# Jamie725/Multimodal-Object-Detection-via-Probabilistic-Ensembling

Measured on AMD Instinct MI355X. Metric: RGB+T frame-pairs/sec (FLIR-aligned 640x512, two R101-FPN detectors + ProbEn), higher is better.
Workload: dtype f16; 1 GPU; configs[2]: FLIR RGB + thermal two-detector ProbEn (probEn/v-avg), batch 32 per GPU, R101-FPN x2, 640x512 -> 800x1000 (padded 800x1024), K=3, random-init weights; batch_per_gpu=32, input_residency=frames resident in HBM before the timed region (no H2D inside it), schedule=two detector streams, staggered by res3, batches back to back

## Files before the change

include/proben_hip.h:

```cpp
#ifndef PROBEN_HIP_H
#define PROBEN_HIP_H

#include <stddef.h>
#include <stdint.h>

#ifdef __cplusplus
extern "C" {
#endif

#define PE_OK 0
#define PE_ERR_INVALID_ARG (-1)
#define PE_ERR_UNSUPPORTED (-2)
#define PE_ERR_HIP (-3)

#define PE_SCORE_PROBEN 0
#define PE_SCORE_AVG 1
#define PE_SCORE_MAX 2
#define PE_SCORE_PROBEN_BINARY 3
#define PE_SCORE_PROBEN_LOGP 4
#define PE_BOX_VAVG 0
#define PE_BOX_SAVG 1
#define PE_BOX_AVG 2
#define PE_BOX_ARGMAX 3

// ... 87 lines not shown
#define PE_POOL_NLL_MAX_BLOCKS 1024
int pe_proben_fuse_batch_pooled(const double* boxes, const double* scores, const double* log_probs,
                                const double* variances, const int32_t* classes, const int32_t* row_source,
                                const int32_t* offsets, const int32_t* row_counts, const int32_t* passthrough, int32_t num_images,
                                int32_t num_classes, int32_t max_rows_per_image, int32_t box_mode, double iou_thresh, double frame_w,
                                double frame_h, const double* log_prior,
                                const double* pool_weights,
                                int32_t num_detectors, double* out_boxes, float* out_scores, float* out_classes, int32_t* out_keep,
                                int32_t* out_counts, int32_t* out_cluster , void* stream);
int pe_proben_pack_pooled(const float* const* det_boxes_host, const float* const* det_scores_host,
                          const int32_t* const* det_classes_host, const float* const* det_probs_host,
                          const float* const* det_logits_host, const float* const* det_vars_host,
                          const int32_t* const* det_counts_host, const double* temperatures_host,
                          const double* var_scales_host , int32_t num_detectors, int32_t num_images,
                          int32_t det_stride, int32_t num_classes, int32_t max_class, int32_t row_stride, double* out_boxes,
                          double* out_scores, double* out_probs, double* out_log_probs , double* out_vars,
                          int32_t* out_classes, int32_t* out_offsets, int32_t* out_counts, int32_t* out_single_source,
                          int32_t* out_source, void* stream);
int pe_pool_nll(const double* log_probs, const int32_t* row_source, int64_t num_rows, int32_t num_columns,
                const int32_t* member_rows, int64_t num_members, const int32_t* cluster_offsets, const int32_t* labels,
                int32_t num_clusters, const double* log_prior , const double* weights_host, int32_t num_candidates,
                int32_t num_detectors, double* workspace, double* out, int32_t* out_flags , void* stream);

int pe_proben_fuse_batch_posterior(const double* boxes, const double* scores, const double* log_probs,
                                   const double* variances, const int32_t* classes, const int32_t* row_source,
                                   const int32_t* offsets, const int32_t* row_counts, const int32_t* passthrough, int32_t num_images,
                                   int32_t num_classes, int32_t max_rows_per_image, int32_t box_mode, double iou_thresh, double frame_w,
                                   double frame_h, const double* log_prior,
                                   const double* pool_weights,
                                   int32_t num_detectors, double* out_boxes, float* out_scores, float* out_classes, int32_t* out_keep,
                                   int32_t* out_counts, int32_t* out_cluster ,
                                   double* out_log_posterior , double* out_vars ,
                                   int32_t* out_members , void* stream);

#define PE_PRESENCE_MAX_DETECTORS 4
#define PE_BIAS_NLL_MAX_COLUMNS 16
#define PE_BIAS_NLL_MAX_BLOCKS 1024
int pe_proben_fuse_batch_presence(const double* boxes, const double* scores, const double* log_probs,
                                  const double* variances, const int32_t* classes, const int32_t* row_source,
                                  const int32_t* offsets, const int32_t* row_counts, const int32_t* passthrough, int32_t num_images,
                                  int32_t num_classes, int32_t max_rows_per_image, int32_t box_mode, double iou_thresh, double frame_w,
                                  double frame_h, const double* log_prior,
                                  const double* pool_weights,
                                  const double* presence,
                                  int32_t num_detectors, double* out_boxes, float* out_scores, float* out_classes, int32_t* out_keep,
                                  int32_t* out_counts, int32_t* out_cluster ,
                                  double* out_log_posterior , double* out_vars ,
                                  int32_t* out_members ,
                                  int32_t* out_pattern , void* stream);
int pe_bias_nll(const double* base, const int32_t* labels, int32_t num_clusters, int32_t num_columns, const double* candidates_host,
                int32_t num_candidates, double* workspace, double* out, int32_t* out_flags , void* stream);

#define PE_BOX_CORR_MAX_DETECTORS PE_PRESENCE_MAX_DETECTORS
#define PE_BOX_PAIR_MAX_BLOCKS 1024
int pe_box_gls_batch(const double* boxes, const double* variances, const int32_t* row_source, const int32_t* cluster,
                     const int32_t* offsets, const int32_t* row_counts , const int32_t* counts, int32_t num_images,
                     int32_t max_rows_per_image, const double* correlation, int32_t num_detectors, double* out_boxes ,
                     double* out_vars , void* stream);
int pe_box_pair_stats(const double* boxes, const double* variances, const int32_t* row_source, int64_t num_rows,
                      const int32_t* member_rows, int64_t num_members, const int32_t* cluster_offsets, const int32_t* cluster_match,
                      int32_t num_clusters, const double* gt_boxes, int64_t num_gt, int32_t num_detectors,
                      const float* bbox_reg_weights_host , double* workspace, double* out ,
                      int32_t* out_flags , void* stream);

int pe_conv2d_nhwc_f16(const void* input, const void* weight, const float* bias, const void* residual,
                       void* output, int32_t N, int32_t H, int32_t W, int32_t Cin, int32_t Cout,
                       int32_t kernel, int32_t stride, int32_t relu, int32_t residual_mode,
                       int32_t res_h, int32_t res_w, int32_t out_f32, int32_t cout_store,
                       int32_t out_stride, void* stream);

int pe_conv_wd_supported(int32_t kernel, int32_t stride, int32_t H, int32_t W, int32_t Cin, int32_t Cout);
int pe_conv_wd_pack_weights(const void* weight, void* packed, int32_t Cout, int32_t Cin, int32_t kernel, void* stream);
int pe_conv3x3_wd_f16(const void* input, const void* packed_weight, const float* bias, void* output, int32_t N,
                      int32_t H, int32_t W, int32_t Cin, int32_t Cout, int32_t relu, int32_t out_stride, void* stream);
int pe_conv_wd_pack_tail(const void* weight, void* packed, int32_t tail_cout, int32_t C, void* stream);
int pe_bottleneck_tail_wd_f16(const void* input, const void* packed_weight3x3, const float* bias3x3, const void* packed_tail,
                              const float* tail_bias, const void* residual, void* output, int32_t N, int32_t H, int32_t W,
                              int32_t Cin, int32_t tail_cout, void* stream);
size_t pe_bneck64_packed_bytes(int32_t has_shortcut_conv, int32_t has_next);
int pe_bneck64_pack(const void* w2, const void* w3, const void* wsc, const void* w1n, void* packed, void* stream);
int pe_bneck64_f16(const void* t1, const void* shortcut_src, const void* packed, const float* bias2, const float* bias3,
                   const float* bias_sc, const float* bias1n, void* out, void* t1_next, int32_t N, int32_t H, int32_t W,
                   int32_t has_shortcut_conv, int32_t has_next, void* stream);
int pe_conv_wd_pack_head(const void* head_weight, void* packed, int32_t rows, int32_t C, void* stream);
int pe_conv3x3_wd_rpn_head_f16(const void* input, const void* packed_weight, const float* bias, const void* packed_head,
                               const float* head_bias16, float* head_out, int32_t N, int32_t H, int32_t W, int32_t Cin,
                               void* stream);

int pe_preprocess_pack(const void* src, int32_t src_kind, int32_t src_h, int32_t src_w, int32_t src_c,
                       int32_t ch0, int32_t nch, int32_t flip_rgb, int32_t dst_h, int32_t dst_w,
                       int32_t pad_h, int32_t pad_w, const float* mean_host, const float* std_host,
                       void* dst, void* stream);
int pe_preprocess_pack_batch(const void* src, int32_t num_images, int32_t src_kind, int32_t src_h, int32_t src_w,
                             int32_t src_c, int32_t ch0, int32_t nch, int32_t flip_rgb, int32_t dst_h, int32_t dst_w,
                             int32_t pad_h, int32_t pad_w, const float* mean_host, const float* std_host, void* dst,
                             void* stream);
int pe_preprocess_pack_pil_u8(const void* src, int32_t num_images, int32_t src_h, int32_t src_w, int32_t src_c,
                              int32_t ch0, int32_t nch, int32_t flip_rgb, int32_t dst_h, int32_t dst_w, int32_t pad_h,
                              int32_t pad_w, const float* mean_host, const float* std_host, const int32_t* xtab,
                              int32_t xk, const int32_t* ytab, int32_t yk, void* dst, void* stream);
int pe_fusion_input_pack(const void* thermal, const void* rgb, int32_t num_images, int32_t th_h, int32_t th_w, int32_t rgb_h,
                         int32_t rgb_w, int32_t ch0, int32_t nch, int32_t dst_h, int32_t dst_w, int32_t pad_h, int32_t pad_w,
                         int32_t pad_multiple, const float* mean_host, const float* std_host, void* dst, void* stream);
int pe_maxpool3x3s2_nhwc(const void* in, void* out, int32_t N, int32_t H, int32_t W, int32_t C, void* stream);
int pe_subsample2_nhwc(const void* in, void* out, int32_t N, int32_t H, int32_t W, int32_t C, void* stream);
int pe_stem_conv7x7_maxpool_f16(const void* x, const void* w_packed, const float* bias, void* out, int32_t N,
                                int32_t H, int32_t W, void* stream);

#define PE_NMS_TRICK 0
#define PE_NMS_CLASS 1
size_t pe_nms_scratch_bytes(int32_t B, int32_t n_max);
int pe_nms_batched(const float* boxes, const float* scores, const int32_t* idxs, const int32_t* counts,
                   const uint8_t* valid, int32_t B, int32_t n_max, float iou_thresh, int32_t mode,
                   int32_t max_out, int32_t* out_keep, int32_t* out_counts, void* scratch,
                   size_t scratch_bytes, void* stream);

int pe_rpn_select_topk(const float* const* level_heads_host, const int32_t* level_hw_host,
                       const int32_t* level_stride_host, const float* cell_anchors_host,
                       int32_t num_levels, int32_t N, int32_t head_stride, int32_t pre_nms_topk,
                       const int32_t* image_hw, float scale_clamp, float* cand_boxes, float* cand_scores,
                       int32_t* cand_level, uint8_t* cand_valid, int32_t cand_per_image, void* scratch,
                       size_t scratch_bytes, void* stream);
size_t pe_rpn_scratch_bytes(const int32_t* level_hw_host, int32_t num_levels, int32_t N);
int pe_gather_boxes(const float* boxes, const float* scores, const int32_t* keep, const int32_t* counts,
                    int32_t N, int32_t n_in, int32_t max_out, float* out_boxes, float* out_scores,
                    void* stream);

int pe_box2box_apply_deltas(const float* deltas, const float* boxes, int32_t N, int32_t k, const float* weights_host,
                            float scale_clamp, float* out, void* stream);
int pe_grid_anchors(const float* cell_anchors, int32_t num_cell_anchors, int32_t H, int32_t W, int32_t stride,
                    float offset, float* out, void* stream);

int pe_sgd_momentum_f32(float* params, const float* grads, float* momentum_buf, void* fp16_shadow, int64_t n, float lr,
                        float momentum, float weight_decay, float grad_scale, int32_t first_step, void* stream);

int pe_roi_align_nhwc(const void* const* feats_host, const int32_t* feat_hw_host, const float* scales_host,
                      int32_t num_levels, int32_t N, int32_t C, int32_t dtype, const float* rois,
                      int32_t rois_have_batch_index, int32_t num_rois, int32_t per_image,
                      const int32_t* counts, int32_t pooled_h, int32_t pooled_w, int32_t sampling_ratio,
                      int32_t aligned, void* output, int32_t* out_level, void* stream);

int pe_roi_align_nhwc_sorted(const void* const* feats_host, const int32_t* feat_hw_host, const float* scales_host,
                             int32_t num_levels, int32_t N, int32_t C, int32_t dtype, const float* boxes, int32_t per_image,
                             const int32_t* counts, int32_t pooled_h, int32_t pooled_w, int32_t sampling_ratio,
                             int32_t aligned, void* output, int32_t* out_level, int32_t* order_workspace, void* stream);

int pe_roi_align_backward_nhwc(const void* grad_output, int32_t dtype, const int32_t* feat_hw_host, const float* scales_host,
                               int32_t num_levels, int32_t N, int32_t C, const float* rois, int32_t rois_have_batch_index,
                               int32_t num_rois, int32_t per_image, const int32_t* counts, int32_t pooled_h,
                               int32_t pooled_w, int32_t sampling_ratio, int32_t aligned, float* const* grad_feats_host,
                               void* stream);

int pe_boxhead_candidates(const float* head, int32_t head_stride, int32_t N, int32_t per_image,
                          int32_t num_classes, const int32_t* prop_counts, const float* proposals,
                          const int32_t* image_hw, const float* reg_weights_host, float scale_clamp,
                          float score_thresh, int32_t cand_max, float* cand_boxes, float* cand_scores,
                          int32_t* cand_class, int32_t* cand_rows, int32_t* cand_counts, int32_t* cand_total,
                          float* probs, void* stream);
int pe_boxhead_finalize(const float* head, int32_t head_stride, int32_t N, int32_t per_image,
                        int32_t num_classes, int32_t cand_max, int32_t max_det, int32_t fix_vars,
                        const float* probs, const float* cand_boxes, const float* cand_scores,
                        const int32_t* cand_class, const int32_t* cand_rows, const int32_t* keep,
                        const int32_t* keep_counts, const int32_t* image_hw, const int32_t* out_hw,
                        float* det_boxes, float* det_scores, int32_t* det_classes, float* det_logits,
                        float* det_probs, float* det_vars, int32_t* det_rows, int32_t* det_counts,
                        void* stream);
// ... 12 lines not shown
```

multimodal-object-detection-via-probabilistic-ensembling_amd/_lib.py:

```python
import ctypes
import os

import torch

_PKG = os.path.dirname(os.path.abspath(__file__))
LIB_PATH = os.path.join(_PKG, "libproben_hip.so")
_lib = None

c_void_p, c_int, c_double, c_float = ctypes.c_void_p, ctypes.c_int32, ctypes.c_double, ctypes.c_float
c_size_t = ctypes.c_size_t

SIGNATURES = {
    "pe_version": [],
    "pe_proben_pack_detections": [c_void_p] * 6 + [c_int] * 6 + [c_void_p] * 9,
    "pe_proben_pack_logits": [c_void_p] * 6 + [c_int] * 6 + [c_void_p] * 9,
    "pe_proben_pack_log_posteriors": [c_void_p] * 6 + [c_int] * 6 + [c_void_p] * 10,
    "pe_log_softmax": [c_void_p, ctypes.c_int64, c_int, c_double, c_void_p, c_void_p],
    "pe_proben_fuse_batch_logp": [c_void_p] * 8 + [c_int] * 4 + [c_double] * 3 + [c_void_p] * 6 + [c_void_p],
    "pe_calibrated_softmax": [c_void_p, ctypes.c_int64, c_int, c_double, c_void_p, c_void_p],
    "pe_temperature_nll": [c_void_p, c_void_p, ctypes.c_int64, c_int, c_void_p, c_int, c_void_p, c_void_p, c_void_p, c_void_p],
    "pe_match_ground_truth": [c_void_p] * 6 + [c_int, c_double, c_int] + [c_void_p] * 4,
    "pe_variance_stats": [c_void_p] * 4 + [ctypes.c_int64, ctypes.c_int64, c_void_p, c_double] + [c_void_p] * 4,
    "pe_proben_pack_calibrated": [c_void_p] * 9 + [c_int] * 6 + [c_void_p] * 10,
    "pe_proben_fuse_batch_pooled": [c_void_p] * 9 + [c_int] * 4 + [c_double] * 3 + [c_void_p] * 2 + [c_int] + [c_void_p] * 6 + [c_void_p],
    "pe_proben_fuse_batch_posterior": [c_void_p] * 9 + [c_int] * 4 + [c_double] * 3 + [c_void_p] * 2 + [c_int] + [c_void_p] * 9 + [c_void_p],
    "pe_proben_fuse_batch_presence": [c_void_p] * 9 + [c_int] * 4 + [c_double] * 3 + [c_void_p] * 3 + [c_int] + [c_void_p] * 10 + [c_void_p],
    "pe_bias_nll": [c_void_p, c_void_p, c_int, c_int, c_void_p, c_int, c_void_p, c_void_p, c_void_p, c_void_p],
    "pe_box_gls_batch": [c_void_p] * 7 + [c_int, c_int, c_void_p, c_int] + [c_void_p] * 3,
    "pe_box_pair_stats": [c_void_p] * 3 + [ctypes.c_int64, c_void_p, ctypes.c_int64, c_void_p, c_void_p, c_int, c_void_p, ctypes.c_int64,
                          c_int] + [c_void_p] * 5,
    "pe_proben_pack_pooled": [c_void_p] * 9 + [c_int] * 6 + [c_void_p] * 11,
    "pe_pool_nll": [c_void_p, c_void_p, ctypes.c_int64, c_int, c_void_p, ctypes.c_int64, c_void_p, c_void_p, c_int, c_void_p, c_void_p,
                    c_int, c_int, c_void_p, c_void_p, c_void_p, c_void_p],
    "pe_reliability_logits": [c_void_p] * 3 + [ctypes.c_int64, c_int, c_double, c_int] + [c_void_p] * 5,
    "pe_reliability_scores": [c_void_p] * 2 + [ctypes.c_int64, c_int] + [c_void_p] * 5,
    "pe_proben_fuse_batch": [c_void_p] * 8 + [c_int] * 5 + [c_double] * 3 + [c_void_p] * 5 + [c_void_p],
    "pe_conv2d_nhwc_f16": [c_void_p] * 5 + [c_int] * 14 + [c_void_p],
    "pe_conv_wd_supported": [c_int] * 6,
    "pe_conv_wd_pack_weights": [c_void_p] * 2 + [c_int] * 3 + [c_void_p],
    "pe_conv3x3_wd_f16": [c_void_p] * 4 + [c_int] * 7 + [c_void_p],
    "pe_conv_wd_pack_tail": [c_void_p] * 2 + [c_int] * 2 + [c_void_p],
    "pe_bottleneck_tail_wd_f16": [c_void_p] * 7 + [c_int] * 5 + [c_void_p],
    "pe_bneck64_packed_bytes": [c_int] * 2,
    "pe_bneck64_pack": [c_void_p] * 6,
    "pe_bneck64_f16": [c_void_p] * 9 + [c_int] * 5 + [c_void_p],
    "pe_conv_wd_pack_head": [c_void_p] * 2 + [c_int] * 2 + [c_void_p],
    "pe_conv3x3_wd_rpn_head_f16": [c_void_p] * 6 + [c_int] * 4 + [c_void_p],
    "pe_preprocess_pack": [c_void_p] + [c_int] * 11 + [c_void_p] * 4,
    "pe_preprocess_pack_batch": [c_void_p] + [c_int] * 12 + [c_void_p] * 4,
    "pe_preprocess_pack_pil_u8": [c_void_p] + [c_int] * 11 + [c_void_p] * 2 + [c_void_p, c_int, c_void_p, c_int] + [c_void_p] * 2,
    "pe_fusion_input_pack": [c_void_p] * 2 + [c_int] * 12 + [c_void_p] * 4,
    "pe_maxpool3x3s2_nhwc": [c_void_p] * 2 + [c_int] * 4 + [c_void_p],
    "pe_subsample2_nhwc": [c_void_p] * 2 + [c_int] * 4 + [c_void_p],
    "pe_stem_conv7x7_maxpool_f16": [c_void_p] * 4 + [c_int] * 3 + [c_void_p],
    "pe_nms_scratch_bytes": [c_int, c_int],
    "pe_nms_batched": [c_void_p] * 5 + [c_int, c_int, c_float, c_int, c_int] + [c_void_p] * 3 + [c_size_t, c_void_p],
    "pe_rpn_select_topk": [c_void_p] * 4 + [c_int] * 4 + [c_void_p, c_float] + [c_void_p] * 4 + [c_int, c_void_p, c_size_t, c_void_p],
    "pe_rpn_scratch_bytes": [c_void_p, c_int, c_int],
    "pe_box2box_apply_deltas": [c_void_p] * 2 + [c_int] * 2 + [c_void_p, c_float, c_void_p, c_void_p],
    "pe_grid_anchors": [c_void_p, c_int, c_int, c_int, c_int, c_float, c_void_p, c_void_p],
    "pe_gather_boxes": [c_void_p] * 4 + [c_int] * 3 + [c_void_p] * 3,
    "pe_roi_align_nhwc": [c_void_p] * 3 + [c_int] * 4 + [c_void_p] + [c_int] * 3 + [c_void_p] + [c_int] * 4 + [c_void_p] * 3,
    "pe_roi_align_nhwc_sorted": [c_void_p] * 3 + [c_int] * 4 + [c_void_p] + [c_int] + [c_void_p] + [c_int] * 4 + [c_void_p] * 4,
    "pe_sgd_momentum_f32": [c_void_p] * 4 + [ctypes.c_int64] + [ctypes.c_float] * 4 + [c_int, c_void_p],
    "pe_roi_align_backward_nhwc": [c_void_p, c_int, c_void_p, c_void_p, c_int, c_int, c_int, c_void_p, c_int, c_int, c_int, c_void_p, c_int, c_int, c_int, c_int, c_void_p, c_void_p],
    "pe_boxhead_candidates": [c_void_p, c_int, c_int, c_int, c_int] + [c_void_p] * 4 + [c_float, c_float, c_int] + [c_void_p] * 8,
    "pe_cocoeval_bbox": [c_void_p] * 6 + [ctypes.c_int64] + [c_void_p] * 4 + [ctypes.c_int64, c_int, c_int, c_void_p, c_int,
                         c_void_p, c_int, c_void_p, c_int, c_void_p, c_int, c_int, c_void_p, c_void_p],
    "pe_boxhead_finalize": [c_void_p] + [c_int] * 7 + [c_void_p] * 18,
}
_RESTYPE = {"pe_last_error": ctypes.c_char_p, "pe_nms_scratch_bytes": ctypes.c_size_t, "pe_rpn_scratch_bytes": ctypes.c_size_t,
             "pe_bneck64_packed_bytes": ctypes.c_size_t}


TEST_HOOKS = {"pe_test_set_conv_policy": [c_int, c_int], "pe_test_set_wd9_mode": [c_int], "pe_test_wd9_takes": [c_int] * 5, "pe_test_wd9_head_takes": [c_int] * 3, "pe_test_set_wd9_wgs": [c_int, c_int], "pe_test_set_ring_wgs": [c_int], "pe_test_set_roi_fast": [c_int], "pe_test_set_nms_presorted": [c_int]}


class HipLibraryError(RuntimeError):
    pass


def lib():
    global _lib
    if _lib is None:
        if not os.path.exists(LIB_PATH):
            raise HipLibraryError(
                f"{LIB_PATH} is missing: run `python -c 'import __graft_entry__ as g; g.build()'` "
                "(hipcc --offload-arch=gfx950).  proben_amd has no CPU fallback.")
        L = ctypes.CDLL(LIB_PATH)
        L.pe_last_error.restype = ctypes.c_char_p
        L.pe_last_error.argtypes = []
        for name, args in SIGNATURES.items():
            fn = getattr(L, name)
            fn.argtypes = args
            fn.restype = _RESTYPE.get(name, ctypes.c_int)
        _lib = L
    return _lib


LAB_HOOKS = {"pe_test_set_ring_ablation": [c_int]}


def test_hooks():
    L = lib()
    for name, args in LAB_HOOKS.items():
        if hasattr(L, name):
            getattr(L, name).argtypes, getattr(L, name).restype = args, ctypes.c_int
    for name, args in TEST_HOOKS.items():
        fn = getattr(L, name)
        fn.argtypes, fn.restype = args, ctypes.c_int
    return L


def check(status, what):
    if status != 0:
        raise HipLibraryError(f"{what} failed ({status}): {lib().pe_last_error().decode()}")


def require_cuda(*tensors):
    for t in tensors:
        if t is not None and not t.is_cuda:
            raise HipLibraryError("proben_amd kernels need device tensors (MODEL.DEVICE=cuda); got a CPU tensor. "
                                  "There is no CPU fallback in the product path.")


def ptr(t):
    if t is None:
        return None
# ... 7 lines not shown
```

multimodal-object-detection-via-probabilistic-ensembling_amd/layers.py:

```python
import ctypes

import numpy as np
import torch

from . import _lib

_scratch = {}
PROFILE = None


def _get_scratch(nbytes, device):
    key = (device.index, torch.cuda.current_stream().cuda_stream)
    buf = _scratch.get(key)
    if buf is None or buf.numel() < nbytes:
        buf = torch.empty(int(nbytes * 1.25) + 1024, dtype=torch.uint8, device=device)
        _scratch[key] = buf
    return buf


def nms_batched_raw(boxes, scores, idxs, counts, valid, iou_threshold, mode, max_out):
    _lib.require_cuda(boxes, scores)
    B, n = scores.shape
    dev = boxes.device
    keep = torch.empty((B, max_out), dtype=torch.int32, device=dev)
# ... 185 lines not shown

def conv3x3_wd(x, packed, bias, cout, *, relu=False, out=None, out_stride=0):
    _lib.require_cuda(x, packed, bias)
    N, H, W, Cin = x.shape
    if out is None:
        out = torch.empty((N, H, W, out_stride or cout), dtype=torch.float16, device=x.device)
    st = _lib.lib().pe_conv3x3_wd_f16(_lib.ptr(x), _lib.ptr(packed), _lib.ptr(bias), _lib.ptr(out), N, H, W, Cin, cout,
                                      int(relu), int(out_stride), _lib.stream())
    _lib.check(st, "pe_conv3x3_wd_f16")
    if PROFILE is not None:
        M = N * H * W
        wd9 = _lib.test_hooks().pe_test_wd9_takes(N, H, W, Cin, cout)
        PROFILE.append({"variant": "conv3x3_wd9_kernel<8, 4, 5, 0>" if wd9 else "conv3x3_wd_kernel<1, 4, 4, 4, 0, 0>",
                        "shape": f"N{N} {H}x{W} Cin{Cin} Cout{cout} k3 s1 res0 f320",
                        "flops": 2.0 * M * cout * 9 * Cin, "bytes": float(M * Cin * 2 + cout * 9 * Cin * 2 + M * cout * 2),
                        "replay": (lambda: conv3x3_wd(x, packed, bias, cout, relu=relu, out=out, out_stride=out_stride))})
    return out


def conv_wd_pack_tail(weight2d):
    _lib.require_cuda(weight2d)
    cout, C = weight2d.shape
    assert weight2d.dtype == torch.float16 and weight2d.is_contiguous()
    packed = torch.empty(cout * C, dtype=torch.float16, device=weight2d.device)
    _lib.check(_lib.lib().pe_conv_wd_pack_tail(_lib.ptr(weight2d), _lib.ptr(packed), cout, C, _lib.stream()), "pe_conv_wd_pack_tail")
    return packed


def bottleneck_tail_wd(x, packed3x3, bias3x3, packed_tail, tail_bias, residual, tail_cout, out=None):
    _lib.require_cuda(x, packed3x3, bias3x3, packed_tail, tail_bias)
    N, H, W, Cin = x.shape
    if out is None:
        out = torch.empty((N, H, W, tail_cout), dtype=torch.float16, device=x.device)
    if residual is not None:
        assert residual.is_contiguous() and tuple(residual.shape) == (N, H, W, tail_cout)
    st = _lib.lib().pe_bottleneck_tail_wd_f16(_lib.ptr(x), _lib.ptr(packed3x3), _lib.ptr(bias3x3), _lib.ptr(packed_tail), _lib.ptr(tail_bias),
                                              _lib.ptr(residual), _lib.ptr(out), N, H, W, Cin, int(tail_cout), _lib.stream())
    _lib.check(st, "pe_bottleneck_tail_wd_f16")
    if PROFILE is not None:
        M = N * H * W
        PROFILE.append({"variant": "conv3x3_wd_kernel<1, 4, 4, 4, 0, 2>",
                        "shape": f"N{N} {H}x{W} Cin{Cin} Cout256->{tail_cout} k3+k1 s1 res{int(residual is not None)} f320",
                        "flops": 2.0 * M * 256 * 9 * Cin + 2.0 * M * tail_cout * 256,
                        "bytes": float(M * Cin * 2 + 256 * 9 * Cin * 2 + tail_cout * 256 * 2 + M * tail_cout * 2 * (2 if residual is not None else 1)),
                        "replay": (lambda: bottleneck_tail_wd(x, packed3x3, bias3x3, packed_tail, tail_bias, residual, tail_cout, out=out))})
    return out


def bneck64_pack(w2, w3, wsc=None, w1n=None):
    _lib.require_cuda(w2, w3)
    assert tuple(w2.shape) == (64, 3, 3, 64) and w3.numel() == 256 * 64 and w2.dtype == torch.float16
    for w in (w2, w3, wsc, w1n):
        assert w is None or (w.is_contiguous() and w.dtype == torch.float16 and w.numel() in (64 * 576, 256 * 64))
    nbytes = _lib.lib().pe_bneck64_packed_bytes(int(wsc is not None), int(w1n is not None))
    packed = torch.empty(nbytes // 2, dtype=torch.float16, device=w2.device)
    _lib.check(_lib.lib().pe_bneck64_pack(_lib.ptr(w2), _lib.ptr(w3), _lib.ptr(wsc), _lib.ptr(w1n), _lib.ptr(packed), _lib.stream()), "pe_bneck64_pack")
    return packed


def bneck64(t1, shortcut_src, packed, bias2, bias3, bias_sc=None, bias1n=None, out=None, t1_next=None):
    _lib.require_cuda(t1, shortcut_src, packed, bias2, bias3)
    N, H, W, C = t1.shape
    has_sc, has_next = bias_sc is not None, bias1n is not None
    assert C == 64 and t1.is_contiguous() and shortcut_src.is_contiguous() and t1.dtype == torch.float16
    assert tuple(shortcut_src.shape) == (N, H, W, 64 if has_sc else 256)
    assert packed.numel() * 2 == _lib.lib().pe_bneck64_packed_bytes(int(has_sc), int(has_next)), "packed stream does not match the requested stages"
    if out is None:
        out = torch.empty((N, H, W, 256), dtype=torch.float16, device=t1.device)
    if has_next and t1_next is None:
        t1_next = torch.empty((N, H, W, 64), dtype=torch.float16, device=t1.device)
    st = _lib.lib().pe_bneck64_f16(_lib.ptr(t1), _lib.ptr(shortcut_src), _lib.ptr(packed), _lib.ptr(bias2), _lib.ptr(bias3), _lib.ptr(bias_sc),
                                   _lib.ptr(bias1n), _lib.ptr(out), _lib.ptr(t1_next if has_next else None), N, H, W, int(has_sc), int(has_next),
                                   _lib.stream())
    _lib.check(st, "pe_bneck64_f16")
    if PROFILE is not None:
        M = N * H * W
        PROFILE.append({"variant": f"bneck64_kernel<{int(has_sc)}, {int(has_next)}>", "shape": f"N{N} {H}x{W} 64->64->256{'+sc' if has_sc else '+id'}{'->64' if has_next else ''} f320",
                        "flops": 2.0 * M * 64 * (576 + 256 + (64 if has_sc else 0) + (256 if has_next else 0)),
                        "bytes": float(M * 2 * (64 + (64 if has_sc else 256) + 256 + (64 if has_next else 0)) + packed.numel() * 2),
                        "replay": (lambda: bneck64(t1, shortcut_src, packed, bias2, bias3, bias_sc, bias1n, out=out, t1_next=t1_next))})
    return out, (t1_next if has_next else None)


def conv_wd_pack_head(weight2d):
    _lib.require_cuda(weight2d)
    rows, C = weight2d.shape
    assert weight2d.dtype == torch.float16 and weight2d.is_contiguous()
    packed = torch.empty(4 * 4 * 64 * 8, dtype=torch.float16, device=weight2d.device)
    _lib.check(_lib.lib().pe_conv_wd_pack_head(_lib.ptr(weight2d), _lib.ptr(packed), rows, C, _lib.stream()), "pe_conv_wd_pack_head")
    return packed


def conv3x3_wd_rpn_head(x, packed, bias, packed_head, head_bias16, out=None):
    _lib.require_cuda(x, packed, bias, packed_head, head_bias16)
    N, H, W, Cin = x.shape
    if out is None:
        out = torch.empty((N, H, W, 16), dtype=torch.float32, device=x.device)
    st = _lib.lib().pe_conv3x3_wd_rpn_head_f16(_lib.ptr(x), _lib.ptr(packed), _lib.ptr(bias), _lib.ptr(packed_head), _lib.ptr(head_bias16),
                                               _lib.ptr(out), N, H, W, Cin, _lib.stream())
    _lib.check(st, "pe_conv3x3_wd_rpn_head_f16")
    if PROFILE is not None:
        M = N * H * W
        wd9 = _lib.test_hooks().pe_test_wd9_head_takes(N, H, W)
        PROFILE.append({"variant": "conv3x3_wd9_kernel<8, 4, 9, 1>" if wd9 else "conv3x3_wd_kernel<1, 4, 4, 4, 0, 1>",
                        "shape": f"N{N} {H}x{W} Cin{Cin} Cout256+head k3 s1 res0 f321",
                        "flops": 2.0 * M * 256 * 9 * Cin + 2.0 * M * 15 * 256, "bytes": float(M * Cin * 2 + 256 * 9 * Cin * 2 + M * 15 * 4),
                        "replay": (lambda: conv3x3_wd_rpn_head(x, packed, bias, packed_head, head_bias16, out=out))})
    return out


DEFAULT_CONV_POLICY = 329


def conv_variant_name(M, Cout, kernel, K=0, *, stride=1, residual_mode=0, out_f32=False, has_bias=True, cout_store=0, out_stride=0, in_pixels=None):
    bn = 64 if Cout <= 64 else 128
    if kernel == 7:
        return "conv_igemm_kernel<128, 64, 2>"
    if kernel == 1:
        ring = (stride in (1, 2) and not out_f32 and has_bias and Cout % 256 == 0
                and (K >= (512 if stride == 1 else 256) if residual_mode == 0 else (stride == 1 and K >= 128 and M * Cout * 2 < 2 ** 31))
                and (cout_store or Cout) == Cout and (in_pixels or M) * K * 2 < 2 ** 31 and Cout * K * 2 < 2 ** 31 and M * (out_stride or Cout) * 2 < 2 ** 31)
        if ring:
            return "conv1x1_ring_kernel"
        if K >= 4096 and Cout % 256 == 0 and ((M + 255) // 256) * (Cout // 256) >= 224:
            return "conv_big_kernel<0>"
        return f"conv_igemm2_kernel<128, {bn}, 0, 1>"
    if bn == 64:
        return "conv3x3rb_kernel<128, 64>"
    big = ((M + 255) // 256) * ((Cout + 127) // 128) >= 512
    return f"conv3x3rb_kernel<{256 if big else 128}, 128>"


def linear_f16(x, weight, bias, *, relu=False, out_f32=False, cout_store=0, out_stride=0):
    M, K = x.shape
    y = conv2d_nhwc(x.view(M, 1, 1, K), weight.view(weight.shape[0], 1, 1, K), bias, kernel=1, relu=relu,
                    out_f32=out_f32, cout_store=cout_store, out_stride=out_stride)
    return y.view(M, -1)


def maxpool3x3s2_nhwc(x):
    N, H, W, C = x.shape
    out = torch.empty((N, (H - 1) // 2 + 1, (W - 1) // 2 + 1, C), dtype=torch.float16, device=x.device)
    _lib.check(_lib.lib().pe_maxpool3x3s2_nhwc(_lib.ptr(x), _lib.ptr(out), N, H, W, C, _lib.stream()), "pe_maxpool3x3s2_nhwc")
    return out


def stem_conv_pool(x, weight_shifted, bias):
    N, H, W, C = x.shape
    assert C == 4 and tuple(weight_shifted.shape) == (64, 7, 8, 4) and x.dtype == torch.float16
    out = torch.empty((N, H // 4, W // 4, 64), dtype=torch.float16, device=x.device)
    _lib.check(_lib.lib().pe_stem_conv7x7_maxpool_f16(_lib.ptr(x), _lib.ptr(weight_shifted), _lib.ptr(bias), _lib.ptr(out),
                                                      N, H, W, _lib.stream()), "pe_stem_conv7x7_maxpool_f16")
    return out


def subsample2_nhwc(x):
    N, H, W, C = x.shape
    out = torch.empty((N, (H - 1) // 2 + 1, (W - 1) // 2 + 1, C), dtype=torch.float16, device=x.device)
    _lib.check(_lib.lib().pe_subsample2_nhwc(_lib.ptr(x), _lib.ptr(out), N, H, W, C, _lib.stream()), "pe_subsample2_nhwc")
    return out


def preprocess_pack(src, dst, *, src_kind, ch0, nch, flip_rgb, dst_hw, mean, std):
    _lib.require_cuda(src, dst)
    if src_kind == 2:
        c, h, w = src.shape
# ... 67 lines not shown
```

multimodal-object-detection-via-probabilistic-ensembling_amd/rcnn.py:

```python
import ctypes
import math
from dataclasses import dataclass

import torch

from . import _lib
from . import layers as L
from .data import PairFrames
from .structures import Boxes, Instances
from .weights import STAGE_BLOCKS, PackedDetector

SCALE_CLAMP = math.log(1000.0 / 16)


@dataclass
class DetectorConfig:
    num_classes: int = 3
    input_format: str = "BGR"
    pixel_mean: tuple = (103.53, 116.28, 123.675)
    pixel_std: tuple = (1.0, 1.0, 1.0)
    anchor_sizes: tuple = (32, 64, 128, 256, 512)
    aspect_ratios: tuple = (0.5, 1.0, 2.0)
    pre_nms_topk: int = 1000
    post_nms_topk: int = 1000
    rpn_nms_thresh: float = 0.7
    score_thresh: float = 0.5
    nms_thresh: float = 0.5
    detections_per_image: int = 100
    min_size_test: int = 800
    max_size_test: int = 1333
    output_logits: bool = True
    enable_gaussian_nll: bool = True
    fix_vars: bool = False
    size_divisibility: int = 32

    @property
    def in_channels(self):
        return {"BGR": 3, "RGB": 3, "BGRT": 4, "BGRTTT": 6}[self.input_format]


def cell_anchor_table(sizes, ratios):
    out = []
    for s in sizes:
        area = float(s) ** 2.0
        for r in ratios:
            w = math.sqrt(area / r)
            h = r * w
            out += [-w / 2.0, -h / 2.0, w / 2.0, h / 2.0]
    return out


class GeneralizedRCNN:
    def __init__(self, cfg: DetectorConfig, state_dict, device="cuda"):
        if not torch.cuda.is_available():
            raise _lib.HipLibraryError("GeneralizedRCNN (MODEL.DEVICE=cuda) needs an MI355X; there is no CPU fallback "
                                       "in proben_amd (the CPU restatement lives in oracle/ for testing only).")
        _lib.lib()
        self.cfg = cfg
        self.device = torch.device(device)
        self.w = PackedDetector(state_dict, device, cfg.num_classes)
        self.depth = self.w.depth
        assert len(cfg.aspect_ratios) == 3, "kernels assume 3 anchors per cell"
        self._cells = (ctypes.c_float * (len(cfg.anchor_sizes) * 12))(*cell_anchor_table(cfg.anchor_sizes, cfg.aspect_ratios))
        self._reg_w = (ctypes.c_float * 4)(10.0, 10.0, 5.0, 5.0)
        self.training = False
        self.use_wd = True
        self.fuse_tails = True
        self.fuse_res2 = True

    def eval(self):
        return self

    def load_state_dict(self, state_dict, strict=True):
        w = PackedDetector(state_dict, self.device, self.cfg.num_classes)
        assert w.depth == self.depth or not strict, f"state dict is ResNet-{w.depth}, model was built as ResNet-{self.depth}"
        self.w, self.depth = w, w.depth
        return self

    def to(self, device):
        assert torch.device(device).type == "cuda", "proben_amd.GeneralizedRCNN lives on the GPU (no CPU fallback)"
        return self

    def _conv(self, x, name, **kw):
        w, b = self.w.convs[name]
        if kw.get("kernel") == 3 and name in self.w.wd and self.use_wd and kw.get("residual") is None and x.numel() * 2 < 2 ** 31 \
                and L.conv_wd_supported(3, 1, x.shape[1], x.shape[2], x.shape[3], w.shape[0]):
            return L.conv3x3_wd(x, self.w.wd[name], b, w.shape[0], relu=kw.get("relu", False), out=kw.get("out"),
                                out_stride=kw.get("out_stride", 0))
        return L.conv2d_nhwc(x, w, b, **kw)

    def _bottom_up(self, x, prefix):
        bu = prefix + ".bottom_up"
        if (bu + ".stem.fused") in self.w.convs and x.shape[1] % 4 == 0 and x.shape[2] % 4 == 0:
            x = L.stem_conv_pool(x, *self.w.convs[bu + ".stem.fused"])
        else:
            x = self._conv(x, bu + ".stem.conv1", kernel=7, stride=2, relu=True)
            x = L.maxpool3x3s2_nhwc(x)
        outs = []
        for si, nb in enumerate(STAGE_BLOCKS[self.depth]):
            chain = self.w.chains64.get(f"{bu}.res{si + 2}") if self.fuse_res2 else None
            if chain is not None and si == 0 and len(chain) == nb and x.shape[0] * x.shape[1] * x.shape[2] * 512 < 2 ** 31:
                t1 = self._conv(x, f"{bu}.res2.0.conv1", kernel=1, relu=True)
                src = x
                for blk in chain:
                    src, t1 = L.bneck64(t1, src, blk["packed"], blk["b2"], blk["b3"], blk["bsc"], blk["b1n"])
                x = src
                outs.append(x)
                hook = getattr(self, "stage_hook", None)
                if hook is not None:
                    hook(si + 2)
                continue
            for bi in range(nb):
                p = f"{bu}.res{si + 2}.{bi}"
                stride = 2 if (bi == 0 and si > 0) else 1
                sc = self._conv(x, p + ".shortcut", kernel=1, stride=stride) if (p + ".shortcut") in self.w.convs else x
                o = self._conv(x, p + ".conv1", kernel=1, stride=stride, relu=True)
                tail = self.w.tails.get(p) if self.use_wd and self.fuse_tails else None
                if tail is not None and L.conv_wd_supported(3, 1, o.shape[1], o.shape[2], o.shape[3], 256) \
                        and o.shape[0] * o.shape[1] * o.shape[2] * self.w.convs[p + ".conv3"][0].shape[0] * 2 < 2 ** 31:
                    x = L.bottleneck_tail_wd(o, self.w.wd[p + ".conv2"], self.w.convs[p + ".conv2"][1], tail[0], tail[1], sc,
                                             self.w.convs[p + ".conv3"][0].shape[0])
                    continue
                o = self._conv(o, p + ".conv2", kernel=3, relu=True)
                x = self._conv(o, p + ".conv3", kernel=1, relu=True, residual=sc, residual_mode=1)
            outs.append(x)
            hook = getattr(self, "stage_hook", None)
            if hook is not None:
                hook(si + 2)
        return outs

    def _fpn(self, x, prefix="backbone", outs=None, ch_off=0, ch_total=256):
        res = self._bottom_up(x, prefix)
        feats = [None] * 5
        prev = None
        for i in (5, 4, 3, 2):
            c = res[i - 2]
            if prev is None:
                prev = self._conv(c, f"{prefix}.fpn_lateral{i}", kernel=1)
            else:
                prev = self._conv(c, f"{prefix}.fpn_lateral{i}", kernel=1, residual=prev, residual_mode=2)
            if outs is None:
                feats[i - 2] = self._conv(prev, f"{prefix}.fpn_output{i}", kernel=3)
            else:
                view = outs[i - 2].view(-1)[ch_off:]
                self._conv(prev, f"{prefix}.fpn_output{i}", kernel=3, out=view, out_stride=ch_total)
                feats[i - 2] = outs[i - 2]
        if outs is None:
            feats[4] = L.subsample2_nhwc(feats[3])
        return feats

    def _preprocess(self, images, resize_to=None):
        cfg = self.cfg
        C = cfg.in_channels
        if isinstance(images, PairFrames):
            return self._preprocess_pair(images, resize_to)
        if isinstance(images, torch.Tensor):
            return self._preprocess_batch(images, resize_to)
        sizes, kinds = [], []
        for im in images:
            chw = im.dim() == 3 and im.shape[0] == C and im.dtype == torch.float32 and im.shape[2] != C
            kinds.append(2 if chw else (0 if im.dtype == torch.uint8 else 1))
            h, w = (im.shape[1], im.shape[2]) if chw else (im.shape[0], im.shape[1])
            sizes.append(tuple(resize_to) if (resize_to is not None and not chw) else (h, w))
        d = cfg.size_divisibility
        Hp = (max(s[0] for s in sizes) + d - 1) // d * d
        Wp = (max(s[1] for s in sizes) + d - 1) // d * d
        mean = list(cfg.pixel_mean)
        std = list(cfg.pixel_std) + [cfg.pixel_std[-1]] * (C - len(cfg.pixel_std))
        assert len(mean) == C, f"PIXEL_MEAN needs {C} entries for INPUT.FORMAT {cfg.input_format}"
        N = len(images)
        groups = [(0, min(C, 4))] if C <= 4 else [(0, 3), (3, 3)]
        batches = []
        for ch0, nch in groups:
            x = torch.empty((N, Hp, Wp, 4), dtype=torch.float16, device=self.device)
            sd0 = 0 if ch0 == 3 else ch0
            for i, im in enumerate(images):
                if kinds[i] == 0 and C == 3 and tuple(sizes[i]) != tuple(im.shape[:2]):
                    L.preprocess_pack_pil_u8(im.contiguous(), x[i], ch0=ch0, nch=nch, flip_rgb=False, dst_hw=sizes[i],
                                             mean=mean[ch0:ch0 + nch], std=std[sd0:sd0 + nch])
                    continue
                L.preprocess_pack(im.contiguous(), x[i], src_kind=kinds[i], ch0=ch0, nch=nch, flip_rgb=False,
                                  dst_hw=sizes[i], mean=mean[ch0:ch0 + nch], std=std[sd0:sd0 + nch])
            batches.append(x)
        return batches, sizes

    def _preprocess_batch(self, images, resize_to):
        cfg = self.cfg
        C = cfg.in_channels
        N = images.shape[0]
        chw = images.dtype == torch.float32 and images.shape[1] == C and images.shape[3] != C
        kind = 2 if chw else (0 if images.dtype == torch.uint8 else 1)
        h, w = (images.shape[2], images.shape[3]) if chw else (images.shape[1], images.shape[2])
        size = tuple(resize_to) if (resize_to is not None and not chw) else (h, w)
        d = cfg.size_divisibility
        Hp, Wp = (size[0] + d - 1) // d * d, (size[1] + d - 1) // d * d
        mean = list(cfg.pixel_mean)
        std = list(cfg.pixel_std) + [cfg.pixel_std[-1]] * (C - len(cfg.pixel_std))
        assert len(mean) == C, f"PIXEL_MEAN needs {C} entries for INPUT.FORMAT {cfg.input_format}"
        batches = []
# ... 205 lines not shown
```

Baseline: 987.2 frame-pairs/s.

## Fuse res3 conv3+residual with next block's conv1 in one persistent kernel

Adds a HIP kernel that computes a bottleneck's 1x1 conv3 (128->512) with bias, residual add and ReLU, keeps the 512-channel output tile in LDS, and immediately runs the next block's 1x1 conv1 (512->128) on it. Both outputs are written from the same pass. This avoids re-reading the 512-channel activation from HBM and drops one launch per block pair in res3. In exchange those blocks no longer use the existing fused conv2+conv3 tail, so conv2 runs as a standalone conv and its output makes an extra HBM round trip. The new kernel also runs one 256-thread block per CU with 160 KiB of LDS, which limits latency hiding.

```diff
diff --git a/include/proben_hip.h b/include/proben_hip.h
--- a/include/proben_hip.h
+++ b/include/proben_hip.h
@@ -193,6 +193,9 @@
 int pe_bneck64_f16(const void* t1, const void* shortcut_src, const void* packed, const float* bias2, const float* bias3,
                    const float* bias_sc, const float* bias1n, void* out, void* t1_next, int32_t N, int32_t H, int32_t W,
                    int32_t has_shortcut_conv, int32_t has_next, void* stream);
+int pe_conv1x1_pair_f16(const void* t2, const void* w3, const float* bias3, const void* residual, const void* w1_next,
+                        const float* bias1_next, void* out, void* t1_next, int32_t N, int32_t H, int32_t W, int32_t Cin,
+                        int32_t Cout, int32_t Cnext, void* stream);
 int pe_conv_wd_pack_head(const void* head_weight, void* packed, int32_t rows, int32_t C, void* stream);
 int pe_conv3x3_wd_rpn_head_f16(const void* input, const void* packed_weight, const float* bias, const void* packed_head,
                                const float* head_bias16, float* head_out, int32_t N, int32_t H, int32_t W, int32_t Cin,
diff --git a/multimodal-object-detection-via-probabilistic-ensembling_amd/_lib.py b/multimodal-object-detection-via-probabilistic-ensembling_amd/_lib.py
--- a/multimodal-object-detection-via-probabilistic-ensembling_amd/_lib.py
+++ b/multimodal-object-detection-via-probabilistic-ensembling_amd/_lib.py
@@ -44,6 +44,7 @@
     "pe_bneck64_packed_bytes": [c_int] * 2,
     "pe_bneck64_pack": [c_void_p] * 6,
     "pe_bneck64_f16": [c_void_p] * 9 + [c_int] * 5 + [c_void_p],
+    "pe_conv1x1_pair_f16": [c_void_p] * 8 + [c_int] * 6 + [c_void_p],
     "pe_conv_wd_pack_head": [c_void_p] * 2 + [c_int] * 2 + [c_void_p],
     "pe_conv3x3_wd_rpn_head_f16": [c_void_p] * 6 + [c_int] * 4 + [c_void_p],
     "pe_preprocess_pack": [c_void_p] + [c_int] * 11 + [c_void_p] * 4,
diff --git a/multimodal-object-detection-via-probabilistic-ensembling_amd/csrc/conv1x1_pair.hip b/multimodal-object-detection-via-probabilistic-ensembling_amd/csrc/conv1x1_pair.hip
--- /dev/null
+++ b/multimodal-object-detection-via-probabilistic-ensembling_amd/csrc/conv1x1_pair.hip
@@ -0,0 +1,318 @@
+#include <atomic>
+#include <cstdint>
+
+#include "conv_common.h"
+
+namespace {
+
+typedef int int4v __attribute__((ext_vector_type(4)));
+typedef unsigned uint4v __attribute__((ext_vector_type(4)));
+typedef float float8v __attribute__((ext_vector_type(8)));
+
+constexpr int PR_BM = 64;
+constexpr int PR_K1 = 128, PR_CY = 512, PR_C2 = 128;
+constexpr int PR_SLAB_B = PR_BM * ROW_B;
+constexpr int PR_Y_B = (PR_CY / 64) * PR_SLAB_B;
+constexpr int PR_T_B = (PR_K1 / 64) * PR_SLAB_B;
+constexpr int PR_STAGE_B = PR_Y_B + PR_T_B;
+constexpr int PR_LDS = 2 * PR_STAGE_B;
+constexpr int PR_THREADS = 256;
+constexpr unsigned PR_OOB = 0x80000000u;
+static_assert(PR_LDS == 160 * 1024, "two stages fill the CU's LDS");
+static_assert(PR_BM * PR_C2 * 2 == PR_T_B, "the t1' patch re-uses the t2 slab");
+
+struct PairArgs {
+    const _Float16* t2;
+    const _Float16* w3;
+    const float* b3;
+    const _Float16* res;
+    const _Float16* w1;
+    const float* b1;
+    _Float16* y;
+    _Float16* t1;
+    int M, ntiles;
+};
+
+__device__ __forceinline__ int4v pr_make_rsrc(const void* p, unsigned bytes) {
+    const unsigned long long a = reinterpret_cast<unsigned long long>(p);
+    int4v r;
+    r[0] = __builtin_amdgcn_readfirstlane((int)(a & 0xffffffffu));
+    r[1] = __builtin_amdgcn_readfirstlane((int)((a >> 32) & 0xffffu));
+    r[2] = __builtin_amdgcn_readfirstlane((int)bytes);
+    r[3] = 0x00020000;
+    return r;
+}
+
+__device__ __forceinline__ void pr_dma2(unsigned lds, int4v rsrc, unsigned soff, unsigned v0, unsigned v1) {
+    unsigned keep;
+    lds = __builtin_amdgcn_readfirstlane(lds);
+    soff = __builtin_amdgcn_readfirstlane(soff);
+    asm volatile(
+        "s_mov_b32 %0, m0\n\t"
+        "s_mov_b32 m0, %1\n\t"
+        "s_nop 0\n\t"
+        "buffer_load_dwordx4 %4, %2, %3 offen lds\n\t"
+        "s_add_u32 m0, m0, 0x400\n\t"
+        "s_nop 0\n\t"
+        "buffer_load_dwordx4 %5, %2, %3 offen lds\n\t"
+        "s_mov_b32 m0, %0"
+        : "=&s"(keep)
+        : "s"(lds), "s"(rsrc), "s"(soff), "v"(v0), "v"(v1)
+        : "scc", "memory");
+}
+
+struct PrBias64 { float8v v[8]; };
+struct PrBias32 { float8v v[4]; };
+__device__ __forceinline__ unsigned long long pr_uniform(const float* p) {
+    const unsigned long long a = reinterpret_cast<unsigned long long>(p);
+    const unsigned lo = __builtin_amdgcn_readfirstlane((unsigned)a), hi = __builtin_amdgcn_readfirstlane((unsigned)(a >> 32));
+    return ((unsigned long long)hi << 32) | lo;
+}
+__device__ __forceinline__ void pr_bias_issue(PrBias64& b, const float* p) {
+    asm volatile(
+        "s_load_dwordx8 %0, %8, 0x0\n\ts_load_dwordx8 %1, %8, 0x20\n\ts_load_dwordx8 %2, %8, 0x40\n\ts_load_dwordx8 %3, %8, 0x60\n\t"
+        "s_load_dwordx8 %4, %8, 0x80\n\ts_load_dwordx8 %5, %8, 0xa0\n\ts_load_dwordx8 %6, %8, 0xc0\n\ts_load_dwordx8 %7, %8, 0xe0"
+        : "=&s"(b.v[0]), "=&s"(b.v[1]), "=&s"(b.v[2]), "=&s"(b.v[3]), "=&s"(b.v[4]), "=&s"(b.v[5]), "=&s"(b.v[6]), "=&s"(b.v[7])
+        : "s"(pr_uniform(p)));
+}
+__device__ __forceinline__ void pr_bias_issue(PrBias32& b, const float* p) {
+    asm volatile("s_load_dwordx8 %0, %4, 0x0\n\ts_load_dwordx8 %1, %4, 0x20\n\ts_load_dwordx8 %2, %4, 0x40\n\ts_load_dwordx8 %3, %4, 0x60"
+                 : "=&s"(b.v[0]), "=&s"(b.v[1]), "=&s"(b.v[2]), "=&s"(b.v[3])
+                 : "s"(pr_uniform(p)));
+}
+__device__ __forceinline__ void pr_bias_wait(PrBias64& b) {
+    asm volatile("s_waitcnt lgkmcnt(0)"
+                 : "+s"(b.v[0]), "+s"(b.v[1]), "+s"(b.v[2]), "+s"(b.v[3]), "+s"(b.v[4]), "+s"(b.v[5]), "+s"(b.v[6]), "+s"(b.v[7]));
+}
+__device__ __forceinline__ void pr_bias_wait(PrBias32& b) {
+    asm volatile("s_waitcnt lgkmcnt(0)" : "+s"(b.v[0]), "+s"(b.v[1]), "+s"(b.v[2]), "+s"(b.v[3]));
+}
+
+__device__ __forceinline__ int pr_perm(int i) { return ((i >> 2) & 1) * 16 + (i >> 3) * 4 + (i & 3); }
+
+__global__ __launch_bounds__(PR_THREADS) void conv1x1_pair_kernel(PairArgs a) {
+    extern __shared__ __attribute__((aligned(1024))) unsigned char smem[];
+    typedef __attribute__((address_space(3))) unsigned char lds_byte;
+    const unsigned smem_base = (unsigned)(unsigned long long)(lds_byte*)smem;
+
+    const int tid = threadIdx.x, lane = tid & 63;
+    const int wave = __builtin_amdgcn_readfirstlane(tid >> 6);
+    const int G = gridDim.x;
+    const int tb0 = (int)((long long)blockIdx.x * a.ntiles / G), tb1 = (int)((long long)(blockIdx.x + 1) * a.ntiles / G);
+    if (tb1 <= tb0) return;
+
+    const int frow = lane & 31, fkh = lane >> 5;
+    const int fsw = (frow >> 1) & 7;
+    const int prow = pr_perm(frow);
+    const int lrow = lane >> 3, lp = lane & 7;
+
+    const int4v rs_res = pr_make_rsrc(a.res, (unsigned)a.M * (PR_CY * 2));
+    const int4v rs_t2 = pr_make_rsrc(a.t2, (unsigned)a.M * (PR_K1 * 2));
+    const __amdgpu_buffer_rsrc_t ry = __builtin_amdgcn_make_buffer_rsrc(a.y, 0, a.M * (PR_CY * 2), 0x00020000);
+    const __amdgpu_buffer_rsrc_t rt1 = __builtin_amdgcn_make_buffer_rsrc(a.t1, 0, a.M * (PR_C2 * 2), 0x00020000);
+
+    auto dma_y = [&](int tile, int stage) {
+        unsigned vo[2];
+#pragma unroll
+        for (int g = 0; g < 2; ++g) {
+            const int r = (wave * 2 + g) * 8 + lrow, m = tile * PR_BM + r;
+            vo[g] = m < a.M ? (unsigned)m * (PR_CY * 2) + (unsigned)((lp ^ ((r >> 1) & 7)) * 16) : PR_OOB;
+        }
+        const unsigned lds = smem_base + stage * PR_STAGE_B + wave * 2048;
+#pragma unroll
+        for (int s = 0; s < PR_CY / 64; ++s) pr_dma2(lds + s * PR_SLAB_B, rs_res, (unsigned)(s * 128), vo[0], vo[1]);
+    };
+    auto dma_t = [&](int tile, int stage) {
+        unsigned vo[2];
+#pragma unroll
+        for (int g = 0; g < 2; ++g) {
+            const int r = (wave * 2 + g) * 8 + lrow, m = tile * PR_BM + r;
+            vo[g] = m < a.M ? (unsigned)m * (PR_K1 * 2) + (unsigned)((lp ^ ((r >> 1) & 7)) * 16) : PR_OOB;
+        }
+        const unsigned lds = smem_base + stage * PR_STAGE_B + PR_Y_B + wave * 2048;
+#pragma unroll
+        for (int s = 0; s < PR_K1 / 64; ++s) pr_dma2(lds + s * PR_SLAB_B, rs_t2, (unsigned)(s * 128), vo[0], vo[1]);
+    };
+    dma_y(tb0, 0);
+    dma_t(tb0, 0);
+
+    half8 w3f[4][8], w1f[32];
+#pragma unroll
+    for (int j = 0; j < 4; ++j)
+#pragma unroll
+        for (int ks = 0; ks < 8; ++ks)
+            w3f[j][ks] = *reinterpret_cast<const half8*>(a.w3 + (wave * 128 + j * 32 + prow) * PR_K1 + ks * 16 + fkh * 8);
+#pragma unroll
+    for (int ks = 0; ks < 32; ++ks) w1f[ks] = *reinterpret_cast<const half8*>(a.w1 + (wave * 32 + prow) * PR_CY + ks * 16 + fkh * 8);
+    asm volatile("s_waitcnt vmcnt(0)" ::: "memory");
+    __syncthreads();
+
+    for (int tile = tb0; tile < tb1; ++tile) {
+        const int stage = (tile - tb0) & 1;
+        unsigned char* ys = smem + stage * PR_STAGE_B;
+        unsigned char* ts = ys + PR_Y_B;
+        const int m0 = tile * PR_BM;
+        if (tile + 1 < tb1) dma_y(tile + 1, stage ^ 1);
+
+#pragma unroll
+        for (int jh = 0; jh < 2; ++jh) {
+            PrBias64 bs;
+            pr_bias_issue(bs, a.b3 + wave * 128 + jh * 64);
+#pragma unroll
+            for (int i = 0; i < 2; ++i) {
+                float16v acc[2];
+#pragma unroll
+                for (int j = 0; j < 2; ++j)
+#pragma unroll
+                    for (int e = 0; e < 16; ++e) acc[j][e] = 0.f;
+                const unsigned char* pa = ts + (i * 32 + frow) * ROW_B;
+#pragma unroll
+                for (int ks = 0; ks < 8; ++ks) {
+                    const half8 pf = *reinterpret_cast<const half8*>(pa + (ks >> 2) * PR_SLAB_B + ((((ks & 3) * 2 + fkh) ^ fsw) << 4));
+#pragma unroll
+                    for (int j = 0; j < 2; ++j) acc[j] = __builtin_amdgcn_mfma_f32_32x32x16_f16(w3f[jh * 2 + j][ks], pf, acc[j], 0, 0, 0);
+                }
+                if (i == 0) pr_bias_wait(bs);
+#pragma unroll
+                for (int j = 0; j < 2; ++j) {
+                    const int c0 = j * 4 + fkh * 2;
+                    unsigned char* row = ys + (wave * 2 + jh) * PR_SLAB_B + (i * 32 + frow) * ROW_B;
+                    half8* p0 = reinterpret_cast<half8*>(row + ((c0 ^ fsw) << 4));
+                    half8* p1 = reinterpret_cast<half8*>(row + (((c0 + 1) ^ fsw) << 4));
+                    const half8 r0 = *p0, r1 = *p1;
+                    half8 h0, h1;
+#pragma unroll
+                    for (int e = 0; e < 8; ++e) {
+                        const float b0 = fkh ? bs.v[j * 4 + 2][e] : bs.v[j * 4 + 0][e];
+                        const float b1 = fkh ? bs.v[j * 4 + 3][e] : bs.v[j * 4 + 1][e];
+                        float x0 = acc[j][e] + b0, x1 = acc[j][e + 8] + b1;
+                        x0 += (float)r0[e];
+                        x1 += (float)r1[e];
+                        h0[e] = (_Float16)pe::relu_nan(x0);
+                        h1[e] = (_Float16)pe::relu_nan(x1);
+                    }
+                    *p0 = h0;
+                    *p1 = h1;
+                }
+            }
+        }
+        asm volatile("s_waitcnt lgkmcnt(0)" ::: "memory");
+#pragma unroll
+        for (int q = 0; q < 16; ++q) {
+            const int s = wave * 2 + (q >> 3), r = (q & 7) * 8 + lrow;
+            const half8 v = *reinterpret_cast<const half8*>(ys + s * PR_SLAB_B + (q & 7) * 1024 + lane * 16);
+            const unsigned off = m0 + r < a.M ? (unsigned)(m0 + r) * (PR_CY * 2) + (unsigned)(s * 128 + ((lp ^ ((r >> 1) & 7)) << 4)) : PR_OOB;
+            __builtin_amdgcn_raw_buffer_store_b128(__builtin_bit_cast(uint4v, v), ry, off, 0, 0);
+        }
+        __syncthreads();
+        if (tile + 1 < tb1) dma_t(tile + 1, stage ^ 1);
+
+        PrBias32 bn;
+        pr_bias_issue(bn, a.b1 + wave * 32);
+        float16v acc2[2];
+#pragma unroll
+        for (int i = 0; i < 2; ++i)
+#pragma unroll
+            for (int e = 0; e < 16; ++e) acc2[i][e] = 0.f;
+        {
+            const unsigned char* pa = ys + frow * ROW_B;
+            half8 pf[2][2][2];
+            auto load = [&](int grp, int buf) {
+#pragma unroll
+                for (int kk = 0; kk < 2; ++kk) {
+                    const int ks = grp * 2 + kk;
+                    const int ch = (((ks & 3) * 2 + fkh) ^ fsw) << 4;
+#pragma unroll
+                    for (int i = 0; i < 2; ++i) pf[buf][kk][i] = *reinterpret_cast<const half8*>(pa + (ks >> 2) * PR_SLAB_B + i * 32 * ROW_B + ch);
+                }
+            };
+            load(0, 0);
+#pragma unroll
+            for (int grp = 0; grp < 16; ++grp) {
+                if (grp + 1 < 16) load(grp + 1, (grp + 1) & 1);
+                __builtin_amdgcn_sched_barrier(0);
+#pragma unroll
+                for (int kk = 0; kk < 2; ++kk)
+#pragma unroll
+                    for (int i = 0; i < 2; ++i)
+                        acc2[i] = __builtin_amdgcn_mfma_f32_32x32x16_f16(w1f[grp * 2 + kk], pf[grp & 1][kk][i], acc2[i], 0, 0, 0);
+                __builtin_amdgcn_sched_barrier(0);
+            }
+        }
+        pr_bias_wait(bn);
+#pragma unroll
+        for (int i = 0; i < 2; ++i) {
+            half8 h0, h1;
+#pragma unroll
+            for (int e = 0; e < 8; ++e) {
+                const float b0 = fkh ? bn.v[2][e] : bn.v[0][e];
+                const float b1 = fkh ? bn.v[3][e] : bn.v[1][e];
+                h0[e] = (_Float16)pe::relu_nan(acc2[i][e] + b0);
+                h1[e] = (_Float16)pe::relu_nan(acc2[i][e + 8] + b1);
+            }
+            const int r = i * 32 + frow, c0 = wave * 4 + fkh * 2;
+            *reinterpret_cast<half8*>(ts + r * 256 + ((c0 ^ (r & 15)) << 4)) = h0;
+            *reinterpret_cast<half8*>(ts + r * 256 + (((c0 + 1) ^ (r & 15)) << 4)) = h1;
+        }
+        asm volatile("s_waitcnt vmcnt(0)" ::: "memory");
+        __syncthreads();
+#pragma unroll
+        for (int q = 0; q < 4; ++q) {
+            const int piece = wave * 4 + q, r = piece * 4 + (lane >> 4);
+            const half8 v = *reinterpret_cast<const half8*>(ts + piece * 1024 + lane * 16);
+            const unsigned off = m0 + r < a.M ? (unsigned)(m0 + r) * (PR_C2 * 2) + (unsigned)((((lane & 15) ^ (r & 15))) << 4) : PR_OOB;
+            __builtin_amdgcn_raw_buffer_store_b128(__builtin_bit_cast(uint4v, v), rt1, off, 0, 0);
+        }
+    }
+}
+
+int pair_cu_count() {
+    static std::atomic<int> cached[64];
+    int dev = 0;
+    if (hipGetDevice(&dev) != hipSuccess || dev < 0 || dev >= 64) {
+        pe::set_error("pe_conv1x1_pair_f16: hipGetDevice failed");
+        return 0;
+    }
+    int n = cached[dev].load(std::memory_order_relaxed);
+    if (n == 0) {
+        if (hipDeviceGetAttribute(&n, hipDeviceAttributeMultiprocessorCount, dev) != hipSuccess || n <= 0) {
+            pe::set_error("pe_conv1x1_pair_f16: cannot read the CU count of device %d", dev);
+            return 0;
+        }
+        cached[dev].store(n, std::memory_order_relaxed);
+    }
+    return n;
+}
+
+}
+
+extern "C" int pe_conv1x1_pair_f16(const void* t2, const void* w3, const float* b3, const void* residual, const void* w1_next,
+                                   const float* b1_next, void* out, void* t1_next, int32_t N, int32_t H, int32_t W, int32_t Cin,
+                                   int32_t Cout, int32_t Cnext, void* stream) {
+    PE_CHECK_ARG(t2 && w3 && b3 && residual && w1_next && b1_next && out && t1_next, "pe_conv1x1_pair_f16: null pointer");
+    PE_CHECK_ARG(N > 0 && H > 0 && W > 0, "pe_conv1x1_pair_f16: bad dims");
+    PE_CHECK_ARG(Cin == PR_K1 && Cout == PR_CY && Cnext == PR_C2, "pe_conv1x1_pair_f16: channels must be 128 -> 512 -> 128 (got %d -> %d -> %d)",
+                 Cin, Cout, Cnext);
+    const long long M = (long long)N * H * W;
+    PE_CHECK_ARG(M * PR_CY * 2 < (1ll << 31), "pe_conv1x1_pair_f16: tensors larger than 2 GiB (32-bit buffer offsets)");
+    {
+        const uintptr_t t2_b = (uintptr_t)M * PR_K1 * 2, y_b = (uintptr_t)M * PR_CY * 2, t1_b = (uintptr_t)M * PR_C2 * 2;
+        auto apart = [](const void* p, uintptr_t pb, const void* q, uintptr_t qb) {
+            return (uintptr_t)p + pb <= (uintptr_t)q || (uintptr_t)q + qb <= (uintptr_t)p;
+        };
+        PE_CHECK_ARG(apart(out, y_b, t2, t2_b) && apart(out, y_b, residual, y_b) && apart(t1_next, t1_b, t2, t2_b) &&
+                         apart(t1_next, t1_b, residual, y_b) && apart(out, y_b, t1_next, t1_b),
+                     "pe_conv1x1_pair_f16: out and t1_next must not overlap t2, residual or each other");
+    }
+    PairArgs a{};
+    a.t2 = (const _Float16*)t2; a.w3 = (const _Float16*)w3; a.b3 = b3; a.res = (const _Float16*)residual;
+    a.w1 = (const _Float16*)w1_next; a.b1 = b1_next; a.y = (_Float16*)out; a.t1 = (_Float16*)t1_next;
+    a.M = (int)M; a.ntiles = pe::ceil_div(M, PR_BM);
+    const int cus = pair_cu_count();
+    if (cus <= 0) return PE_ERR_HIP;
+    const int grid = a.ntiles < cus ? a.ntiles : cus;
+    PE_ENSURE_LDS(conv1x1_pair_kernel, (size_t)PR_LDS, "pe_conv1x1_pair_f16");
+    hipLaunchKernelGGL(conv1x1_pair_kernel, dim3(grid), dim3(PR_THREADS), (size_t)PR_LDS, (hipStream_t)stream, a);
+    PE_CHECK_LAUNCH("pe_conv1x1_pair_f16");
+    return PE_OK;
+}
diff --git a/multimodal-object-detection-via-probabilistic-ensembling_amd/layers.py b/multimodal-object-detection-via-probabilistic-ensembling_amd/layers.py
--- a/multimodal-object-detection-via-probabilistic-ensembling_amd/layers.py
+++ b/multimodal-object-detection-via-probabilistic-ensembling_amd/layers.py
@@ -291,6 +291,32 @@
     return out, (t1_next if has_next else None)
 
 
+def conv1x1_pair_supported(cin, cout, cnext, pixels):
+    return (cin, cout, cnext) == (128, 512, 128) and pixels * cout * 2 < 2 ** 31
+
+
+def conv1x1_pair(t2, w3, b3, residual, w1n, b1n, out=None, t1_next=None):
+    _lib.require_cuda(t2, w3, b3, residual, w1n, b1n)
+    N, H, W, Cin = t2.shape
+    Cout, Cnext = w3.shape[0], w1n.shape[0]
+    assert t2.dtype == torch.float16 and residual.dtype == torch.float16 and tuple(residual.shape) == (N, H, W, Cout)
+    assert w3.numel() == Cout * Cin and w1n.numel() == Cnext * Cout and b3.numel() == Cout and b1n.numel() == Cnext
+    if out is None:
+        out = torch.empty((N, H, W, Cout), dtype=torch.float16, device=t2.device)
+    if t1_next is None:
+        t1_next = torch.empty((N, H, W, Cnext), dtype=torch.float16, device=t2.device)
+    st = _lib.lib().pe_conv1x1_pair_f16(_lib.ptr(t2), _lib.ptr(w3), _lib.ptr(b3), _lib.ptr(residual), _lib.ptr(w1n), _lib.ptr(b1n),
+                                        _lib.ptr(out), _lib.ptr(t1_next), N, H, W, Cin, Cout, Cnext, _lib.stream())
+    _lib.check(st, "pe_conv1x1_pair_f16")
+    if PROFILE is not None:
+        M = N * H * W
+        PROFILE.append({"variant": "conv1x1_pair_kernel", "shape": f"N{N} {H}x{W} {Cin}->{Cout}+id->{Cnext} f320",
+                        "flops": 2.0 * M * Cout * (Cin + Cnext),
+                        "bytes": float(M * 2 * (Cin + 2 * Cout + Cnext) + (w3.numel() + w1n.numel()) * 2),
+                        "replay": (lambda: conv1x1_pair(t2, w3, b3, residual, w1n, b1n, out=out, t1_next=t1_next))})
+    return out, t1_next
+
+
 def conv_wd_pack_head(weight2d):
     _lib.require_cuda(weight2d)
     rows, C = weight2d.shape
diff --git a/multimodal-object-detection-via-probabilistic-ensembling_amd/rcnn.py b/multimodal-object-detection-via-probabilistic-ensembling_amd/rcnn.py
--- a/multimodal-object-detection-via-probabilistic-ensembling_amd/rcnn.py
+++ b/multimodal-object-detection-via-probabilistic-ensembling_amd/rcnn.py
@@ -66,6 +66,7 @@
         self.training = False
         self.use_wd = True
         self.fuse_tails = True
+        self.fuse_pairs = True
         self.fuse_res2 = True
 
     def eval(self):
@@ -110,11 +111,20 @@
                 if hook is not None:
                     hook(si + 2)
                 continue
+            t1 = None
             for bi in range(nb):
                 p = f"{bu}.res{si + 2}.{bi}"
                 stride = 2 if (bi == 0 and si > 0) else 1
                 sc = self._conv(x, p + ".shortcut", kernel=1, stride=stride) if (p + ".shortcut") in self.w.convs else x
-                o = self._conv(x, p + ".conv1", kernel=1, stride=stride, relu=True)
+                o = t1 if t1 is not None else self._conv(x, p + ".conv1", kernel=1, stride=stride, relu=True)
+                t1 = None
+                pn = f"{bu}.res{si + 2}.{bi + 1}"
+                if self.fuse_pairs and bi + 1 < nb and (pn + ".shortcut") not in self.w.convs:
+                    (w3, b3), (w1n, b1n) = self.w.convs[p + ".conv3"], self.w.convs[pn + ".conv1"]
+                    if L.conv1x1_pair_supported(w3.shape[-1], w3.shape[0], w1n.shape[0], o.shape[0] * o.shape[1] * o.shape[2]):
+                        o = self._conv(o, p + ".conv2", kernel=3, relu=True)
+                        x, t1 = L.conv1x1_pair(o, w3, b3, sc, w1n, b1n)
+                        continue
                 tail = self.w.tails.get(p) if self.use_wd and self.fuse_tails else None
                 if tail is not None and L.conv_wd_supported(3, 1, o.shape[1], o.shape[2], o.shape[3], 256) \
                         and o.shape[0] * o.shape[1] * o.shape[2] * self.w.convs[p + ".conv3"][0].shape[0] * 2 < 2 ** 31:
```

Measured after the change: 1002 frame-pairs/s (median of 6 runs). 1.02x the previous value.
